# lbcb-sci/raven

Hardware: AMD Instinct MI355X
Metric: read Gbase/s through overlap+polish (higher is better)
Workload: dtype u32

## Files before the change

raven_amd/csrc/engine.h:

```cpp
#pragma once

#include <atomic>
#include <functional>
#include <memory>
#include <mutex>
#include <string>
#include <vector>

#include "common.h"

namespace rvn {

constexpr int kSketchTile = 1024;
constexpr int kMaxWindow = 256;

inline u64 next_reads_serial() {
  static std::atomic<u64> counter{0};
  return ++counter;
}

using BufFn = std::function<void(DevBuf&)>;
template <typename G>
void release_bufs(G& g) {
  g.for_each_buf([](DevBuf& b) { b.release(); });
// ... 34 lines not shown
  u64 m = 0;
  u64 u = 0;
  int table_bits = 0;
  int shift = 0;
  DevBuf s_val[2];
  DevBuf s_org[2];
  int cur = 0;
  DevBuf u_val;
  DevBuf u_start;
  DevBuf table;
  DevBuf direct;
  bool direct_built = false;
  u32 occurrence = 0xFFFFFFFFu;
  bool table_built = false;
  bool has_query_flags = false;
  bool all_query = false;
  u32 first = 0, last = 0;
  void for_each_buf(const BufFn& f) {
    f(s_val[0]), f(s_val[1]), f(s_org[0]), f(s_org[1]), f(u_val), f(u_start), f(table), f(direct);
  }
};

struct MapOut {
  u32 first = 0, last = 0;
  u64 n_query = 0;
  u64 n_matches = 0;
  u64 n_intervals = 0;
  u64 n_overlaps = 0;
  DevBuf ovl;
  DevBuf ovl_read_off;
  DevBuf filtered;
  bool has_anchors = false;
  DevBuf anchors;
  DevBuf anchor_off;
  DevBuf anchor_cnt;
  void for_each_buf(const BufFn& f) { f(ovl), f(ovl_read_off), f(filtered), f(anchors), f(anchor_off), f(anchor_cnt); }
};

struct StageTimes {
  enum { kSketch, kSort, kIndex, kFilter, kQuery, kMatch, kSegSort, kIntervals, kChain, kCompact, kMerge, kPile,
         kTruncate, kNum };
  double ms[kNum] = {};
  u64 launches[kNum] = {};
};

struct PileState;
struct PileRegion;
struct ResolveState;

struct EngineOptions {
  long long nw_budget_mb = 0;
  long long nw_group_walk = 0;
  long long nw_stripe_lanes = 0;
  long long ed_wide_lanes = 0;
  long long index_direct_min_keys = 0;
  long long poa_rows_min_windows = -1;
  long long io_threads = 0;
  long long io_slab_mb = 0;
  long long io_ring = 0;
  long long io_zlib = 0;
  long long arena_mb = 0;
  long long arena_margin_mb = 0;
  long long no_arena = 0;
  long long release_always = 0;
  long long polish_join = 0;
  long long polish_sketch_cache_mb = -1;
};
const char* engine_option_names();
long long* engine_option(EngineOptions& o, const char* name);

struct Engine;

struct SharedScratch {
  DevBuf tmp_a, tmp_b, tmp_c, tmp_d, tmp_e, tmp_f, scan_tmp, sort_tmp;
  void for_each_buf(const BufFn& f) {
    f(tmp_a), f(tmp_b), f(tmp_c), f(tmp_d), f(tmp_e), f(tmp_f), f(scan_tmp), f(sort_tmp);
  }
  void release() { release_bufs(*this); }
};

struct IoState {
  DevBuf text[2];
  std::vector<std::pair<std::unique_ptr<PinBuf>, bool>> pin;
  void for_each_buf(const BufFn& f) { f(text[0]), f(text[1]); }
  void release() { release_bufs(*this); }
};
struct LoadStats {
  u64 n_sequences = 0, n_bases = 0;
  int has_quality = 0;
  double parse_s = 0, device_s = 0, total_s = 0;
  u32 inflate_threads = 0, members = 0;
  int streaming = 0, restarted = 0;
};
void reads_load(Engine& e, const std::string& path, ReadsDev& R, std::vector<std::string>& names, LoadStats& st);

struct SketchState {
  Index index;
  Sketch index_sketch, query_sketch, raw_sketch;
  struct QueryReady {
    bool valid = false;
    u32 first = 0, last = 0;
    bool minhash = false;
  } query_ready;
  u64 join_query_count = 0;
  bool shard_sketch_minhash = false;
  DevBuf foreign_val, foreign_org;
// ... 61 lines not shown
void chain_allow_big_lds();

struct EditDistanceState {
  DevBuf cnt, sort, todo;
  void for_each_buf(const BufFn& f) { f(cnt), f(sort), f(todo); }
  void release() { release_bufs(*this); }
};
void edit_distance_batch(Engine& e, const ReadsDev& r, const u32* h_pairs, u32 n_pairs, u32* h_out, double* kernel_ms,
                         u64* cells);
void edit_distance_dev(Engine& e, const ReadsDev& r, const u32* d_pairs, u32 n_pairs, u32* d_out, const u32* d_kmax = nullptr,
                       bool wide_sweep = false);

struct PoaState {
  DevBuf scratch, scratch2;
  DevBuf sched, redo_w, redo_i;
  int mode = 0;
  u32 fallback_windows = 0;
  u32 fullmatrix_windows = 0;
  u32 wide_windows = 0;
  u32 narrow_windows = 0;
  unsigned long long phase_cycles[8] = {};
  u64 cells_full = 0, cells_band = 0, calls = 0;
  void for_each_buf(const BufFn& f) { f(scratch), f(scratch2), f(sched), f(redo_w), f(redo_i); }
  void release() { release_bufs(*this); }
};
void poa_consensus_batch(Engine& e, const u8* h_codes, const u8* h_quals, const u64* h_layer_off, const u32* h_begins,
                         const u32* h_ends, const u32* h_has_qual, const u32* h_win_off, u32 n_windows, int m, int n,
                         int g, int trim, u8* h_out, const u64* h_out_off, u32* h_out_len, u32* h_status,
                         double* device_ms);

void poa_banded_emulate(const u8* h_codes, const u8* h_quals, const u64* h_layer_off, const u32* h_begins,
                        const u32* h_ends, const u32* h_has_qual, const u32* h_win_off, u32 n_windows, int m, int n, int g,
                        int trim, u8* h_out, const u64* h_out_off, u32* h_out_len, u32* h_status, int variant);

struct PolishStats {
  u64 n_overlaps = 0, n_reads_used = 0, n_layers = 0, n_windows = 0, n_polished_windows = 0, n_failed_windows = 0;
  u64 n_dropped_layers = 0;
  double poa_ms = 0;
  double map_ms = 0, host_ms = 0, total_ms = 0;
  double align_ms = 0;
  u64 n_aligned = 0, n_align_retries = 0, align_band_cells = 0, align_store_bytes = 0;
};

struct NwStats {
  u64 n_aligned = 0, n_retries = 0, n_unaligned = 0, n_batches = 0;
  u64 band_cells = 0, sum_distance = 0, store_bytes = 0;
  double ms = 0;
};
struct NwState {
  struct Set {
    DevBuf hs, ck;
  } sets[4];
  DevBuf strip, jobs, res;
  double rate = -1.0;
  NwStats last;
  hipStream_t streams[5] = {};
  hipEvent_t ev[5] = {};
  hipStream_t side[3] = {};
  hipEvent_t side_ev[4] = {};
  void for_each_buf(const BufFn& f) {
    for (Set& s : sets) f(s.hs), f(s.ck);
    f(strip), f(jobs), f(res);
  }
  void release() { release_bufs(*this); }
  void open();
  void close();
  ~NwState() { close(); }
};
struct NwJob;
struct NwWindowRec;
struct NwPathSlots {
  std::vector<std::unique_ptr<DevBuf>> blocks;
  std::vector<u64> slot_end;
};
void nw_breakpoints(Engine& e, const ReadsDev& T, const ReadsDev& R, std::vector<NwJob>& jobs, u32 w, NwWindowRec* d_recs,
                    u64 n_recs, NwStats& st, std::vector<u32>* distances = nullptr, NwPathSlots* path = nullptr);
struct NwPaths {
  u32 n = 0, n_not_aligned = 0;
  u64 n_runs = 0, n_ops = 0;
  std::vector<u32> distances;
  DevBuf run_off, runs, op_off;
  double device_ms = 0;
};
void nw_align_paths(Engine& e, const ReadsDev& T, const ReadsDev& Q, std::vector<NwJob>& jobs, NwPaths& out);
void nw_paths_expand(Engine& e, const NwPaths& p, u8* d_ops);
int nw_breakpoints_host(const u64* t_words, u32 t_len, const u64* r_words, u32 r_len, u32 t_begin, u32 n, u32 q_begin, u32 m,
                        int rc, u32 w, u32 k, int force_R, NwWindowRec* recs, u32* distance, u32* band);
struct ShardState {
  DevBuf hist, off, ptrs;
  void for_each_buf(const BufFn& f) { f(hist), f(off), f(ptrs); }
  void release() { release_bufs(*this); }
};
void shard_split_minimizers(Engine& e, const u64* d_val, const u64* d_org, u64 n, u32 world, u64* d_val_out, u64* d_org_out,
                            u64* counts );
void shard_split_overlaps(Engine& e, const Overlap* d_ovl, u64 n, const u32* bounds , u32 world, u32 self,
                          Overlap* d_out, u64* counts );
u64 shard_count_flagged(Engine& e, const u64* d_org, u64 n);
void shard_adjacent_diff(Engine& e, const u64* d_seg, u64 n, u64* d_cnt);
void shard_regroup(Engine& e, u32 world, const u64* const* d_cnt, const u64* const* d_grp, const u64* const* d_pos,
                   const u64* n_src , u32 n_reads, u64* d_seg, u64* d_grp_out, u64* d_pos_out);
void shard_lhs_offsets(Engine& e, const Overlap* d_ovl, u64 n, u32 n_reads, u32* d_off);
struct PolishDirectOut {
  u8* out;
  const u64* off;
  u64* len;
};
struct PolishState {
  DevBuf best, best_t, idmap, recs, keep, win_cnt, win_off, win_fill, win_meta, first_window, keys, lays_tmp, lays, wins, out,
      len, status, ok, cons_off, stitched, quals, qual_off, misc;
  DevBuf tval, torg;
  struct KeptSketch {
    u32 first = 0, last = 0;
    Sketch sk;
  };
  u64 sketch_owner = 0;
// ... 357 lines not shown
```

raven_amd/csrc/engine.hip:

```cpp
#include <chrono>
#include <memory>

#include "abi.h"
#include "poa.h"

using namespace rvn;

static_assert(sizeof(rvn_overlap) == sizeof(rvn::Overlap), "overlap layout");

namespace {

thread_local std::string g_err;

const char* kStageNames[StageTimes::kNum] = {"sketch", "sort", "index", "filter", "query_sketch", "match",
                                             "seg_sort", "intervals", "chain", "compact", "merge", "pile",
                                             "truncate"};

}

namespace rvn {

void set_last_error(const std::string& msg) { g_err = msg; }
const std::string& last_error() { return g_err; }

// ... 16 lines not shown
    }
    Sketch& is = e.sketch.index_sketch;
    if (join && minhash) {
      sketch_minhash(e, r, e.sketch.raw_sketch, is);
      ix.all_query = true;
    } else if (!minhash) {
      is.val.swap(e.sketch.raw_sketch.val);
      is.org.swap(e.sketch.raw_sketch.org);
      is.read_off.swap(e.sketch.raw_sketch.read_off);
      is.first = first;
      is.last = last;
      is.count = e.sketch.raw_sketch.count;
      e.sketch.raw_sketch.count = 0;
      raw_handed_over = true;
    } else if (prefetch_query) {
      const Sketch& qs = e.sketch.query_sketch;
      const size_t vb = e.val64 ? 8 : 4;
      is.first = first;
      is.last = last;
      is.count = qs.count;
      is.val.reserve((qs.count + 1) * vb);
      is.org.reserve((qs.count + 1) * 8);
      if (qs.count) {
        RVN_HIP(hipMemcpyAsync(is.val.ptr, qs.val.ptr, qs.count * vb, hipMemcpyDeviceToDevice, e.stream));
        RVN_HIP(hipMemcpyAsync(is.org.ptr, qs.org.ptr, qs.count * 8, hipMemcpyDeviceToDevice, e.stream));
      }
    } else {
      sketch_minhash(e, r, e.sketch.raw_sketch, is);
    }
    t.stop();
  }
  for (u32 i = first; i < last; ++i) e.c_index_bases += r.h_len[i];
  e.c_index_min += e.sketch.index_sketch.count;
  index_build(e, e.sketch.index_sketch, !(e.sketch.index.has_query_flags || e.sketch.index.all_query));
  e.c_index_keys += e.sketch.index.u;
  if (raw_handed_over) {
    if (e.sketch.raw_sketch.val.cap < e.sketch.index_sketch.val.cap) e.sketch.raw_sketch.val.swap(e.sketch.index_sketch.val);
    if (e.sketch.raw_sketch.org.cap < e.sketch.index_sketch.org.cap) e.sketch.raw_sketch.org.swap(e.sketch.index_sketch.org);
  }
}

void fetch_values(Engine& e, const DevBuf& val, u64 n, u64* values) {
  if (!values || n == 0) return;
  if (e.val64) {
    RVN_HIP(hipMemcpy(values, val.ptr, n * 8, hipMemcpyDeviceToHost));
  } else {
    std::vector<u32> tmp(n);
    RVN_HIP(hipMemcpy(tmp.data(), val.ptr, n * 4, hipMemcpyDeviceToHost));
    for (u64 i = 0; i < n; ++i) values[i] = tmp[i];
  }
}

const char* engine_option_names() {
  return "nw_budget_mb, nw_group_walk, nw_stripe_lanes, ed_wide_lanes, index_direct_min_keys, poa_rows_min_windows, io_threads, io_slab_mb, io_ring, io_zlib, arena_mb, arena_margin_mb, "
         "no_arena, release_always, polish_join, polish_sketch_cache_mb";
}
long long* engine_option(EngineOptions& o, const char* name) {
  const std::string n(name ? name : "");
  if (n == "nw_budget_mb") return &o.nw_budget_mb;
  if (n == "nw_group_walk") return &o.nw_group_walk;
  if (n == "nw_stripe_lanes") return &o.nw_stripe_lanes;
  if (n == "ed_wide_lanes") return &o.ed_wide_lanes;
  if (n == "index_direct_min_keys") return &o.index_direct_min_keys;
  if (n == "poa_rows_min_windows") return &o.poa_rows_min_windows;
  if (n == "io_threads") return &o.io_threads;
  if (n == "io_slab_mb") return &o.io_slab_mb;
  if (n == "io_ring") return &o.io_ring;
  if (n == "io_zlib") return &o.io_zlib;
  if (n == "arena_mb") return &o.arena_mb;
  if (n == "arena_margin_mb") return &o.arena_margin_mb;
  if (n == "no_arena") return &o.no_arena;
  if (n == "release_always") return &o.release_always;
  if (n == "polish_join") return &o.polish_join;
  if (n == "polish_sketch_cache_mb") return &o.polish_sketch_cache_mb;
  return nullptr;
}

void engine_release_scratch(Engine& e) {
  if (e.stream) (void)rvn_stream_sync(e.stream);
  e.for_each_group([](auto& group) { group.release(); });
  delete e.pile_pool;
  e.pile_pool = nullptr;
}
void engine_release_scratch_if_tight(Engine& e, int stage_kind) {
  e.stage_kind = stage_kind;
  size_t free_b = 0, total_b = 0;
  if (hipMemGetInfo(&free_b, &total_b) != hipSuccess) return;
  const bool trace = knob("RVN_DEBUG_MEM") != nullptr;
  if (devpool::active()) {
    const size_t afree = devpool::free_total(), asize = devpool::size();
    const bool tight = afree * 4 < asize || ((e.oom_mask >> stage_kind) & 1u) || e.opt.release_always != 0;
    if (trace)
      std::fprintf(stderr, "[raven_hip] stage entry (kind %d): arena %.1f GB free of %.1f GB, driver %.1f GB free%s\n", stage_kind,
                   afree / 1e9, asize / 1e9, free_b / 1e9, tight ? " -> scratch released" : "");
    if (tight) engine_release_scratch(e);
    return;
  }
  const bool tight = free_b * 4 < total_b || e.opt.release_always != 0;
  if (trace)
    std::fprintf(stderr, "[raven_hip] stage entry (kind %d): %.1f GB free of %.1f GB%s\n", stage_kind, free_b / 1e9, total_b / 1e9,
                 tight ? " -> scratch released, arena started" : "");
  if (!tight) return;
  engine_release_scratch(e);
  if (e.opt.no_arena) return;
  if (hipMemGetInfo(&free_b, &total_b) != hipSuccess) return;
  size_t margin = std::max<size_t>(12ULL << 30, total_b / 16);
  if (e.opt.arena_margin_mb > 0) margin = static_cast<size_t>(e.opt.arena_margin_mb) << 20;
  if (e.opt.arena_mb > 0) margin = free_b > (static_cast<size_t>(e.opt.arena_mb) << 20) ? free_b - (static_cast<size_t>(e.opt.arena_mb) << 20) : free_b;
  if (free_b > margin + (1ULL << 30)) {
    const auto t0 = std::chrono::steady_clock::now();
    const bool ok = devpool::start(free_b - margin);
    if (trace)
      std::fprintf(stderr, "[raven_hip] arena of %.1f GB %s (%.0f ms)\n", (free_b - margin) / 1e9, ok ? "started" : "refused",
                   std::chrono::duration<double, std::milli>(std::chrono::steady_clock::now() - t0).count());
// ... 159 lines not shown
```

raven_amd/csrc/nwpath.hip:

```cpp
#include <algorithm>
#include <mutex>
#include <chrono>
#include <cmath>
#include <cstdio>
#include <cstdlib>
#include <exception>
#include <type_traits>
#include <vector>

#include "engine.h"
#include "nwpath.h"
#include "nwplan.h"
#include "nwsweep.h"
#include "nwtrace.h"
#include "wave.h"

namespace rvn {

namespace {

constexpr int kNwLaneStripCols = 16;
constexpr int kNwGroupLanes = 16;
constexpr u32 kNwGroupWalkMaxJobs = 8192;
constexpr u32 kSideSweepMaxWaves = 2048;
// ... 78 lines not shown
      const int o = __shfl_xor(n_steps_w, off, 64);
      n_steps_w = o > n_steps_w ? o : n_steps_w;
    }
    n_steps_w = __builtin_amdgcn_readfirstlane((n_steps_w + 15) & ~15);
    const int prev = lig == 0 ? gbase + (L > 0 ? L - 1 : 0) : lane - 1;
    const bool st_ok = has && lig < L;
    int n_g = (n_steps + kNwHsSteps - 1) / kNwHsSteps, n_q = n_steps / kNwCkSteps;
    if (STRIPED) {
      n_g = g0 + gps;
      n_q = qc0 + qps;
    }
    const u64 row = static_cast<u64>(L) * R;
    for (int t = t0; t <= n_steps_w; ++t) {
      int x = __shfl(ln.xf, prev, 64);
      if (STRIPED) {
        if (is_top) x = top.x(t);
        if (t == t_hand) sc_hand = ln.sc;
      }
      if (__ballot(ln.has_event(t)) != 0) {
        int sp = __shfl(ln.sc, prev, 64);
        if (STRIPED && is_top) sp = sc_in;
        if (ln.has_event(t)) ln.event(t, x, sp);
      }
      ln.step(t, x);
      if ((t & 15) == 0) {
        const int gi = (t >> 4) - 1;
        if (st_ok && gi < n_g) {
          u32* p = hs_j + static_cast<u64>(gi - g0) * row + static_cast<u64>(lig) * R;
#pragma unroll
          for (int r = 0; r < R; ++r) p[r] = ln.acc[r];
        }
        if ((t & 31) == 0) {
          const int qi = (t >> 5) - 1;
          if (st_ok && qi < n_q) {
            NwPm* p = ck_j + static_cast<u64>(qi - qc0) * row + static_cast<u64>(lig) * R;
#pragma unroll
            for (int r = 0; r < R; ++r) p[r] = NwPm{ln.Pv[r], ln.Mv[r]};
          }
        }
        ln.next_group(t);
        if (STRIPED && is_top) top.next_group(t);
      }
    }
    if (STRIPED && has && lig == lig_hand) hs_j[row * static_cast<u64>(gps)] = static_cast<u32>(sc_hand);
    const u32 res1 = group_max<G>(ln.result);
    if (has && lig == 0 && last) {
      const u32 res = res1 - 1u;
      result[ji] = res;
      status[ji] = (res1 != 0 && res <= k) ? 0u : 2u;
    }
  }
}

template <bool STRIP_LDS, int SC, class Out = NwWindowRec>
__global__ __launch_bounds__(64) void nw_trace_kernel(const NwJob* __restrict__ jobs, const u32* __restrict__ idx, u32 n_idx,
                                                      const u64* __restrict__ t_words, const u64* __restrict__ r_words,
                                                      const u32* __restrict__ hs, const NwPm* __restrict__ ck,
                                                      const u32* __restrict__ result, u32* __restrict__ status, u32 w,
                                                      Out* __restrict__ recs, u64* __restrict__ scratch) {
  __shared__ u64 s_pv[STRIP_LDS ? (SC + 1) * 64 : 1];
  __shared__ u64 s_mv[STRIP_LDS ? (SC + 1) * 64 : 1];
  __builtin_amdgcn_s_setprio(3);
  const u32 q = blockIdx.x * 64 + threadIdx.x;
  if (q >= n_idx) return;
  const u32 ji = idx[q];
  if (status[ji] != 0) return;
  const NwJob J = jobs[ji];
  const NwGeo geo = nw_geo_job(J);
  u64* g_pv = scratch + static_cast<u64>(blockIdx.x) * (2 * kNwStripCols * 64);
  const NwStripMem<64> mem{STRIP_LDS ? s_pv : g_pv, STRIP_LDS ? s_mv : g_pv + kNwStripCols * 64, static_cast<int>(threadIdx.x)};
  if constexpr (std::is_same<Out, u32>::value) {
    NwRunSink sink;
    sink.init(recs + J.bp_off, nw_slot_words(J.k));
    status[ji] = static_cast<u32>(nw_trace_job<64, SC, NwRunSink>(J, geo, t_words, r_words, hs + J.hs, ck + J.ckpt, mem, result[ji], w,
                                                                  nullptr, sink));
  } else {
    status[ji] = static_cast<u32>(nw_trace_job<64, SC>(J, geo, t_words, r_words, hs + J.hs, ck + J.ckpt, mem, result[ji], w, recs));
  }
}

template <int GL, class Out = NwWindowRec>
__global__ __launch_bounds__(64) void nw_trace_group_kernel(const NwJob* __restrict__ jobs, const u32* __restrict__ idx, u32 n_idx,
                                                            const u64* __restrict__ t_words, const u64* __restrict__ r_words,
                                                            const u32* __restrict__ hs, const NwPm* __restrict__ ck,
                                                            const u32* __restrict__ result, u32* __restrict__ status, u32 w,
                                                            Out* __restrict__ recs) {
  constexpr int NG = 64 / GL;
  __shared__ u64 s_pv[kNwStripCols * 64];
  __shared__ u64 s_mv[kNwStripCols * 64];
  __shared__ NwStripHead s_heads[64];
  __builtin_amdgcn_s_setprio(3);
  const int lane = static_cast<int>(threadIdx.x), grp = lane / GL, t = lane % GL;
  const u32 q = blockIdx.x * NG + static_cast<u32>(grp);
  if (q >= n_idx) return;
  const u32 ji = idx[q];
  if (status[ji] != 0) return;
  const NwJob J = jobs[ji];
  const NwGeo geo = nw_geo_job(J);
  constexpr bool kPath = std::is_same<Out, u32>::value;
  NwGroupWalk<64, GL, typename std::conditional<kPath, NwRunSink, NwNoSink>::type> G;
  if constexpr (kPath) {
    NwRunSink sink;
    sink.init(recs + J.bp_off, nw_slot_words(J.k));
    G.init(J, t_words, r_words, NwStripMem<64>{s_pv, s_mv, grp * GL}, s_heads + grp * GL, result[ji], w, nullptr, sink);
  } else {
    G.init(J, t_words, r_words, NwStripMem<64>{s_pv, s_mv, grp * GL}, s_heads + grp * GL, result[ji], w, recs);
  }
  int bad = 0;
  while (!G.done()) {
    G.fill(J, geo, hs + J.hs, ck + J.ckpt, t);
    __threadfence_block();
    __builtin_amdgcn_wave_barrier();
    bad = G.walk_batch(geo, t == 0);
    __threadfence_block();
    __builtin_amdgcn_wave_barrier();
    if (bad) break;
  }
  const int rcode = bad ? 1 : G.wk.finish(t == 0);
  if (t == 0) status[ji] = static_cast<u32>(rcode);
}

template <int R, int G, bool STRIPED = false>
void launch_sweep(Engine& e, hipStream_t s, const NwJob* d_jobs, const u32* d_idx, u32 n_idx, const ReadsDev& T, const ReadsDev& Rd,
                  u32* d_hs, NwPm* d_ck, u32* d_result, u32* d_status, u32* d_next, int stripe = 0) {
  if (n_idx == 0) return;
  constexpr u32 NG = 64 / G;
  const u32 bundles = (n_idx + NG - 1) / NG;
  const u32 per_simd = static_cast<u32>(sweep_waves_per_simd<R>());
  const u32 waves = std::min<u32>(bundles, 256u * 4u * (per_simd > 4 ? per_simd - 2 : per_simd));
  RVN_HIP(hipMemsetAsync(d_next, 0, 4, s));
  RVN_KLAUNCH_ON(kKNwForward, s, (nw_sweep_kernel<R, G, STRIPED><<<(waves + 3) / 4, 256, 0, s>>>(
                               d_jobs, d_idx, n_idx, T.packed.as<u64>(), Rd.packed.as<u64>(), d_hs, d_ck, d_result,
                               d_status, d_next, stripe)));
}


}

void NwState::open() {
  try {
    int prio_least = 0, prio_greatest = 0;
    RVN_HIP(hipDeviceGetStreamPriorityRange(&prio_least, &prio_greatest));
    for (int b = 0; b < 8; ++b) {
      hipStream_t& st2 = b < 5 ? streams[b] : side[b - 5];
      if (b >= 3 && prio_greatest != prio_least) RVN_HIP(hipStreamCreateWithPriority(&st2, hipStreamNonBlocking, prio_greatest));
      else RVN_HIP(hipStreamCreateWithFlags(&st2, hipStreamNonBlocking));
    }
    for (hipEvent_t& x : ev) RVN_HIP(hipEventCreateWithFlags(&x, hipEventDisableTiming));
    for (hipEvent_t& x : side_ev) RVN_HIP(hipEventCreateWithFlags(&x, hipEventDisableTiming));
  } catch (...) {
    close();
    throw;
  }
}
void NwState::close() {
  auto drop = [](auto& all, auto destroy) {
    for (auto& x : all) {
      if (x) (void)destroy(x);
      x = nullptr;
    }
  };
  drop(ev, hipEventDestroy);
  drop(streams, hipStreamDestroy);
  drop(side_ev, hipEventDestroy);
  drop(side, hipStreamDestroy);
}

namespace {

using clk = std::chrono::steady_clock;
double since(clk::time_point t) { return std::chrono::duration<double, std::milli>(clk::now() - t).count(); }

struct WalkGuard {
  Engine& e;
  ~WalkGuard() {
    if (!std::uncaught_exceptions()) return;
    for (hipStream_t st2 : e.nw.streams)
      if (st2) (void)hipStreamSynchronize(st2);
    for (hipStream_t st2 : e.nw.side)
      if (st2) (void)hipStreamSynchronize(st2);
    (void)hipStreamSynchronize(e.stream);
  }
};

u64 nw_budget(Engine& e) {
  size_t free_b = 0, total_b = 0;
  RVN_HIP(hipMemGetInfo(&free_b, &total_b));
  u64 held = 0;
  for (const NwState::Set& set : e.nw.sets) held += set.hs.cap + set.ck.cap;
  u64 budget = std::min<u64>((static_cast<u64>(free_b) + devpool::free_total()) / 4 + held, 64ULL << 30);
  if (e.opt.nw_budget_mb > 0) budget = static_cast<u64>(e.opt.nw_budget_mb) << 20;
  return std::max<u64>(budget, 64ULL << 20);
}

struct NwRun {
  Engine& e;
  const ReadsDev& T;
  const ReadsDev& Rd;
  std::vector<NwJob>& jobs;
  const u32 w;
  NwWindowRec* const d_recs;
  NwPathSlots* const path;
  NwStats& st;
  std::vector<u32>* const distances;
  const hipStream_t s;
  const u32 nj;
  const u64 budget;
  const u32 stripe_lanes;
  const bool trace_lds;
  const int group_walk;
  const bool one_stream, dbg_sync;
  const NwDevArrays dev;
  bool side_pending[3] = {false, false, false};
  bool set_used[4] = {false, false, false, false};
  struct Queued {
    std::vector<u32> order;
    NwPassDev dev;
    bool sweep_only;
    std::vector<u32> res, status;
  };
  std::vector<Queued> queued;
  std::vector<u8> early;
  std::vector<u32> h_result, h_status;
  std::vector<double> rates;
  std::vector<NwObs> obs;
  double h_plan = 0, h_order = 0, h_up = 0, h_res = 0;

  NwRun(Engine& e_, const ReadsDev& T_, const ReadsDev& Rd_, std::vector<NwJob>& jobs_, u32 w_, NwWindowRec* d_recs_, NwPathSlots* path_,
        NwStats& st_, std::vector<u32>* distances_)
      : e(e_), T(T_), Rd(Rd_), jobs(jobs_), w(w_), d_recs(d_recs_), path(path_), st(st_), distances(distances_), s(e_.stream),
        nj(static_cast<u32>(jobs_.size())), budget(nw_budget(e_)),
        stripe_lanes(e_.opt.nw_stripe_lanes > 0 && e_.opt.nw_stripe_lanes < 64 ? static_cast<u32>(e_.opt.nw_stripe_lanes) : 64u),
        trace_lds(!(knob("RVN_NW_TRACE_MEM") && std::atoi(knob("RVN_NW_TRACE_MEM")) == 1)),
        group_walk(static_cast<int>(e_.opt.nw_group_walk)), one_stream(knob("RVN_NW_ONE_STREAM") != nullptr),
        dbg_sync(knob("RVN_NW_DEBUG") && std::atoi(knob("RVN_NW_DEBUG")) >= 2), dev(arrays(e_, nj)), h_result(nj), h_status(nj) {
    rates.reserve(nj);
  }
  static NwDevArrays arrays(Engine& e, u32 nj) {
    const NwDevLayout at = nw_dev_layout(nj);
    NwJob* d_jobs = e.nw.jobs.get<NwJob>(at.n_jobs);
    return nw_dev_arrays(at, d_jobs, e.nw.res.get<u32>(at.n_words));
  }

  bool plan(NwJob& J, u64 k) const { return nw_plan(J, k, stripe_lanes, budget); }

  void join_side() {
    for (int x = 0; x < 3; ++x) {
      if (side_pending[x]) RVN_HIP(hipStreamWaitEvent(s, e.nw.side_ev[x], 0));
      side_pending[x] = false;
    }
  }

  struct ChunkDev {
    const NwPassDev& dev;
    int b;
    u32* hs;
    NwPm* ck;
    u64* d_strip;
    u32* d_slots;
  };

  template <class Out, class... Tail>
  void launch_walk_kernel(void (*kernel)(const NwJob*, const u32*, u32, const u64*, const u64*, const u32*, const NwPm*, const u32*, u32*, u32,
                                         Out*, Tail...),
                          u32 per_block, const ChunkDev& c, Out* d_out, hipStream_t wst, const u32* idx_w, u32 n_w, Tail... tail) {
    RVN_KLAUNCH_ON(kKNwTraceback, wst, (kernel<<<(n_w + per_block - 1) / per_block, 64, 0, wst>>>(
                                           c.dev.jobs, idx_w, n_w, T.packed.as<u64>(), Rd.packed.as<u64>(), c.hs, c.ck, c.dev.res,
                                           c.dev.status, w, d_out, tail...)));
  }
  template <class Out>
  void launch_walk_to(Out* d_out, const ChunkDev& c, hipStream_t wst, const u32* idx_w, u32 n_w) {
    if (group_walk == 2 || (group_walk != 1 && n_w <= kNwGroupWalkMaxJobs)) {
      launch_walk_kernel<Out>(nw_trace_group_kernel<kNwGroupLanes, Out>, 64 / kNwGroupLanes, c, d_out, wst, idx_w, n_w);
    } else if (trace_lds && (group_walk == 3 || (group_walk != 1 && n_w > 64u * 4u * 256u))) {
      launch_walk_kernel<Out, u64*>(nw_trace_kernel<true, kNwLaneStripCols, Out>, 64, c, d_out, wst, idx_w, n_w, nullptr);
    } else if (trace_lds) {
      launch_walk_kernel<Out, u64*>(nw_trace_kernel<true, kNwCkSteps, Out>, 64, c, d_out, wst, idx_w, n_w, nullptr);
    } else {
      launch_walk_kernel<Out, u64*>(nw_trace_kernel<false, kNwCkSteps, Out>, 64, c, d_out, wst, idx_w, n_w,
                                    c.d_strip + static_cast<size_t>(c.b) * ((e.nw.strip.cap / 32) & ~size_t(63)));
    }
  }
  void launch_walk(const ChunkDev& c, hipStream_t wst, const u32* idx_w, u32 n_w) {
    if (path) launch_walk_to(c.d_slots, c, wst, idx_w, n_w);
    else launch_walk_to(d_recs, c, wst, idx_w, n_w);
  }

  template <u32 X>
  void launch_variant(const ChunkDev& c, const NwChunk& C, const u32* idx_c, const bool* side) {
    constexpr int R = static_cast<int>(kNwVariants[X].R), G = static_cast<int>(kNwVariants[X].G);
    const u32 n = nw_count_of(C, X);
    launch_sweep<R, G>(e, side[X] ? e.nw.side[X % 3] : s, c.dev.jobs, idx_c + C.coff[X], n, T, Rd, c.hs, c.ck, c.dev.res, c.dev.status,
                       side[X] ? dev.side_next + X : dev.next);
    if (dbg_sync && n) {
      RVN_HIP(hipStreamSynchronize(s));
      std::fprintf(stderr, "[raven_hip] nw: sweep R=%d G=%d done, %u jobs\n", R, G, n);
    }
  }
  template <u32 X = kLevels - 1>
  void launch_variants(const ChunkDev& c, const NwChunk& C, const u32* idx_c, const bool* side) {
    launch_variant<X>(c, C, idx_c, side);
    if constexpr (X > 0) launch_variants<X - 1>(c, C, idx_c, side);
  }

  void enqueue(const std::vector<u32>& todo, bool sweep_only, NwLayout layout, const NwPassDev& pd, hipStream_t up, std::vector<u32>* left) {
    if (todo.empty()) return;
    auto t_h = clk::now();
    std::vector<u32> order = nw_order(jobs, todo);
    const NwChunks cut = nw_chunks(order, jobs, budget, layout, path && !sweep_only, left);
    const std::vector<NwChunk>& chunks = cut.chunks;
    st.band_cells += cut.band_cells;
    st.store_bytes = std::max<u64>(st.store_bytes, cut.store_bytes);
    for (int b = 0; b < 4; ++b) {
      const NwSetNeed need = nw_set_need(chunks, layout, b);
      if (!need.used) continue;
      (void)e.nw.sets[b].hs.get<u32>(need.hs_w + 4 * 64 * 8 + 16);
      (void)e.nw.sets[b].ck.get<NwPm>(need.ck_e + 16);
    }
    u64* d_strip = nullptr;
    if (!trace_lds) {
      size_t mc = 0;
      for (const NwChunk& C : chunks) mc = std::max(mc, C.c1 - C.c0);
      d_strip = e.nw.strip.get<u64>(static_cast<size_t>((mc + 63) / 64) * 2 * kNwStripCols * 64 * 4 + 64);
    }
    u32* d_slots = nullptr;
    if (path && !sweep_only) {
      path->blocks.emplace_back(new DevBuf());
      d_slots = path->blocks.back()->get<u32>(cut.slot_w + 16);
      for (u32 i : order) path->slot_end[i] = reinterpret_cast<u64>(d_slots + jobs[i].bp_off + nw_slot_words(jobs[i].k) - 1);
    }
    h_order += since(t_h);
    t_h = clk::now();
    if (pd.compact) {
      std::vector<NwJob> hj(order.size());
      std::vector<u32> iota(order.size());
      for (size_t x = 0; x < order.size(); ++x) {
        hj[x] = jobs[order[x]];
        iota[x] = static_cast<u32>(x);
      }
      RVN_HIP(hipMemcpyAsync(pd.jobs, hj.data(), hj.size() * sizeof(NwJob), hipMemcpyHostToDevice, up));
      RVN_HIP(hipMemcpyAsync(pd.idx, iota.data(), iota.size() * 4, hipMemcpyHostToDevice, up));
      RVN_HIP(rvn_stream_sync(up));
    } else {
      RVN_HIP(hipMemcpyAsync(pd.jobs, jobs.data(), static_cast<size_t>(nj) * sizeof(NwJob), hipMemcpyHostToDevice, up));
      RVN_HIP(hipMemcpyAsync(pd.idx, order.data(), order.size() * 4, hipMemcpyHostToDevice, up));
      RVN_HIP(rvn_stream_sync(up));
    }
    h_up += since(t_h);
    for (size_t ci = 0; ci < chunks.size(); ++ci) {
      const NwChunk& C = chunks[ci];
      const int b = nw_set_of(ci, layout);
      const ChunkDev c{pd, b, e.nw.sets[b].hs.as<u32>(), e.nw.sets[b].ck.as<NwPm>(), d_strip, d_slots};
      const u32* idx_c = pd.idx + C.c0;
      const u32 cn = static_cast<u32>(C.c1 - C.c0);
      if (set_used[b]) RVN_HIP(hipStreamWaitEvent(s, e.nw.ev[b], 0));
      hipStream_t ts = one_stream ? s : e.nw.streams[b];
      bool side[kLevels] = {};
      bool side_used[3] = {false, false, false};
      {
        u32 n_levels = 0;
        for (u32 x = 0; x < kLevels; ++x) n_levels += nw_count_of(C, x) ? 1u : 0u;
        if (n_levels >= 2 && !one_stream && !dbg_sync)
          for (u32 x = 0; x < kLevels; ++x) {
            const u32 per_wave = 64 / kNwVariants[x].G;
            const u32 bundles = (nw_count_of(C, x) + per_wave - 1) / per_wave;
            side[x] = nw_count_of(C, x) && bundles <= kSideSweepMaxWaves;
            if (side[x]) side_used[x % 3] = true;
          }
        if (side_used[0] || side_used[1] || side_used[2]) {
          RVN_HIP(hipEventRecord(e.nw.side_ev[3], s));
          for (int y = 0; y < 3; ++y)
            if (side_used[y]) RVN_HIP(hipStreamWaitEvent(e.nw.side[y], e.nw.side_ev[3], 0));
        }
      }
      if (const u32 n_str = nw_count_of(C, kStriped)) {
        const u32* idx_s = idx_c + C.coff[kStriped];
        std::vector<u32> n_stripes(n_str);
        for (u32 x = 0; x < n_str; ++x) n_stripes[x] = static_cast<u32>(nw_geo_job(jobs[order[C.c0 + C.coff[kStriped] + x]]).n_stripes);
        for (u32 stp = 0;; ++stp) {
          u32 n_st = 0;
          while (n_st < n_str && n_stripes[n_st] > stp) ++n_st;
          if (n_st == 0) break;
          launch_sweep<static_cast<int>(kNwStripedVariant.R), static_cast<int>(kNwStripedVariant.G), true>(
              e, s, pd.jobs, idx_s, n_st, T, Rd, c.hs, c.ck, pd.res, pd.status, dev.next, static_cast<int>(stp));
          if (dbg_sync) {
            RVN_HIP(hipStreamSynchronize(s));
            std::fprintf(stderr, "[raven_hip] nw: stripe %u done, %u jobs\n", stp, n_st);
          }
        }
      }
      launch_variants(c, C, idx_c, side);
      for (int y = 0; y < 3; ++y)
        if (side_used[y]) {
          RVN_HIP(hipEventRecord(e.nw.side_ev[y], e.nw.side[y]));
          side_pending[y] = true;
        }
      ++st.n_batches;
      if (sweep_only) continue;
      if (!one_stream) {
        RVN_HIP(hipEventRecord(e.nw.ev[4], s));
        RVN_HIP(hipStreamWaitEvent(ts, e.nw.ev[4], 0));
        for (int y = 0; y < 3; ++y)
          if (side_used[y]) RVN_HIP(hipStreamWaitEvent(ts, e.nw.side_ev[y], 0));
      }
      launch_walk(c, ts, idx_c, cn);
      if (!one_stream) {
        RVN_HIP(hipEventRecord(e.nw.ev[b], ts));
        set_used[b] = true;
      }
      if (dbg_sync) {
        RVN_HIP(hipStreamSynchronize(ts));
        std::fprintf(stderr, "[raven_hip] nw: trace done, %u jobs\n", cn);
      }
    }
    queued.push_back(Queued{std::move(order), pd, sweep_only, {}, {}});
  }

  void collect(std::vector<u32>& again) {
    again.clear();
    join_side();
    for (int b = 0; b < 4; ++b) {
      if (set_used[b]) RVN_HIP(hipStreamWaitEvent(s, e.nw.ev[b], 0));
      set_used[b] = false;
    }
    for (Queued& q : queued) {
      if (q.dev.compact) {
        q.res.resize(q.order.size());
        q.status.resize(q.order.size());
        RVN_HIP(hipMemcpyAsync(q.res.data(), q.dev.res, q.order.size() * 4, hipMemcpyDeviceToHost, s));
        RVN_HIP(hipMemcpyAsync(q.status.data(), q.dev.status, q.order.size() * 4, hipMemcpyDeviceToHost, s));
      }
    }
    RVN_HIP(hipMemcpyAsync(h_result.data(), dev.all.res, static_cast<size_t>(nj) * 4, hipMemcpyDeviceToHost, s));
    RVN_HIP(hipMemcpyAsync(h_status.data(), dev.all.status, static_cast<size_t>(nj) * 4, hipMemcpyDeviceToHost, s));
    RVN_HIP(rvn_stream_sync(s));
    auto t_h = clk::now();
    for (const Queued& q : queued)
      if (q.dev.compact)
        for (size_t x = 0; x < q.order.size(); ++x) {
          h_result[q.order[x]] = q.res[x];
          h_status[q.order[x]] = q.status[x];
        }
    for (size_t qi = 0; qi < queued.size(); ++qi) {
      const Queued& q = queued[qi];
// ... 562 lines not shown
```

raven_amd/csrc/nwplan.h:

```cpp
#pragma once

#include <algorithm>
#include <cmath>
#include <vector>

#include "nwpath.h"

namespace rvn {

struct NwVariant {
  u32 R, G;
};
constexpr NwVariant kNwVariants[] = {{1, 4}, {1, 8}, {1, 16}, {1, 32}, {1, 64}, {2, 64}, {4, 64}, {8, 64}};
constexpr u32 kLevels = sizeof(kNwVariants) / sizeof(kNwVariants[0]);
constexpr NwVariant kNwStripedVariant = kNwVariants[kLevels - 1];
constexpr u32 kNwMaxStripes = 8;
constexpr u32 kStriped = kLevels;
constexpr u32 kClasses = kLevels + 1;
constexpr u32 kHeadMax = 4096;

inline u32 kcap_of(u32 n, u32 m, u32 R, u32 G) {
  const u32 d = n > m ? n - m : m - n;
  const u64 room = static_cast<u64>(G) * (64ULL * R + 1) - 64ULL * R;
  if (room < d) return 0;
// ... 105 lines not shown
    C.c0 = c0;
    size_t c1 = c0;
    while (c1 < order.size()) {
      NwJob& J = jobs[order[c1]];
      const u64 hw = need[c1].hw, ce = need[c1].ce;
      const u64 share = (chunks.empty() && layout != kRotating) ? budget / 12 : budget / 3;
      if (c1 > c0 && (C.hs_w + hw) * 4 + (C.ck_e + ce) * 16 > share) break;
      J.hs = C.hs_w;
      J.ckpt = C.ck_e;
      if (slots) {
        J.bp_off = out.slot_w;
        out.slot_w += nw_slot_words(J.k);
      }
      C.hs_w += hw;
      C.ck_e += ce;
      out.band_cells += need[c1].cells;
      C.coff[need[c1].level + 1]++;
      ++c1;
    }
    u32 run_off = 0, cnt[kClasses];
    for (u32 x = 0; x < kClasses; ++x) cnt[x] = C.coff[x + 1];
    for (int x = static_cast<int>(kClasses) - 1; x >= 0; --x) {
      C.coff[x] = run_off;
      run_off += cnt[x];
    }
    C.coff[kClasses] = run_off;
    C.c1 = c1;
    out.store_bytes = std::max<u64>(out.store_bytes, C.hs_w * 4 + C.ck_e * 16);
    chunks.push_back(C);
    c0 = c1;
    if (layout == kHeadOnly) break;
  }
  if (layout == kHeadOnly && !chunks.empty() && chunks[0].c1 < order.size()) {
    for (size_t x = chunks[0].c1; x < order.size(); ++x) left->push_back(order[x]);
    order.resize(chunks[0].c1);
  }
  return out;
}

struct NwSetNeed {
  bool used;
  u64 hs_w, ck_e;
};
inline NwSetNeed nw_set_need(const std::vector<NwChunk>& chunks, NwLayout layout, int b) {
  NwSetNeed need{false, 0, 0};
  for (size_t ci = 0; ci < chunks.size(); ++ci) {
    if (nw_set_of(ci, layout) != b) continue;
    need.used = true;
    need.hs_w = std::max(need.hs_w, chunks[ci].hs_w);
    need.ck_e = std::max(need.ck_e, chunks[ci].ck_e);
  }
  return need;
}

struct NwObs {
  double len, d;
};
struct NwThresholdModel {
  double mu = -1, va = 0, vb = 0;
  void fit(const std::vector<NwObs>& obs) {
    if (obs.size() < 256) return;
    double sl = 0, sd = 0;
    for (const NwObs& o : obs) {
      sl += o.len;
      sd += o.d;
    }
    mu = sd / sl;
    std::vector<double> zs;
    for (const NwObs& o : obs) zs.push_back(std::fabs(o.d - mu * o.len) / std::sqrt(o.len));
    std::vector<double> zsorted = zs;
    std::sort(zsorted.begin(), zsorted.end());
    const double zcut = zsorted[static_cast<size_t>(zsorted.size() * 0.98)];
    double s11 = 0, s12 = 0, s22 = 0, t1 = 0, t2 = 0, sr = 0, sn = 0;
    for (size_t x = 0; x < obs.size(); ++x) {
      if (zs[x] > zcut) continue;
      const double L = obs[x].len * 1e-3, r2 = (obs[x].d - mu * obs[x].len) * (obs[x].d - mu * obs[x].len);
      s11 += L * L;
      s12 += L * L * L;
      s22 += L * L * L * L;
      t1 += r2 * L;
      t2 += r2 * L * L;
      sr += r2 / L;
      sn += 1;
    }
    const double det = s11 * s22 - s12 * s12;
    double a = -1, b = -1;
    if (det > 1e-9 * s11 * s22) {
      a = (t1 * s22 - t2 * s12) / det;
      b = (t2 * s11 - t1 * s12) / det;
    }
    if (!(a >= 0) || !(b >= 0)) {
      a = sn > 0 ? sr / sn : mu * 1e3;
      b = 0;
    }
    va = std::max(a * 1e-3, 0.25 * mu);
    vb = b * 1e-6;
  }
  u64 threshold(double len, double rate) const {
    const double z = 4.5;
    return mu > 0 ? static_cast<u64>(mu * len + z * std::sqrt(va * len + vb * len * len)) + 6 : static_cast<u64>(rate * len) + 16;
  }
  static u64 pilot_threshold(double len, double rate) { return static_cast<u64>((rate * 1.25 + 0.02) * len) + 16; }
};

inline u32 nw_job_len(const NwJob& J) { return std::max(J.n, J.m); }

// ... 88 lines not shown
```

Baseline: 1.444.

## Pack variable-width R=1 NW sweep jobs into shared wavefronts via host bin-packing

Adds a packed sweep kernel in which one 64-lane wavefront processes several R=1 alignment jobs of different lane widths side by side. A host-side planner sorts the jobs by step count, bin-packs them into bundles by width and uploads a bundle table. By default this applies only to chunks where the per-variant R=1 launches would need more than the side-sweep wave limit. The aim is to cut wasted lanes and per-variant kernel launches from small-width jobs that previously got fixed G-lane groups. In exchange it adds host packing cost, an extra upload, and shuffle and ballot overhead inside the kernel.

```diff
diff --git a/raven_amd/csrc/engine.h b/raven_amd/csrc/engine.h
--- a/raven_amd/csrc/engine.h
+++ b/raven_amd/csrc/engine.h
@@ -110,6 +110,7 @@
   long long nw_budget_mb = 0;
   long long nw_group_walk = 0;
   long long nw_stripe_lanes = 0;
+  long long nw_pack = 1;
   long long ed_wide_lanes = 0;
   long long index_direct_min_keys = 0;
   long long poa_rows_min_windows = -1;
@@ -277,6 +278,7 @@
     DevBuf hs, ck;
   } sets[4];
   DevBuf strip, jobs, res;
+  DevBuf pack;
   double rate = -1.0;
   NwStats last;
   hipStream_t streams[5] = {};
@@ -285,7 +287,7 @@
   hipEvent_t side_ev[4] = {};
   void for_each_buf(const BufFn& f) {
     for (Set& s : sets) f(s.hs), f(s.ck);
-    f(strip), f(jobs), f(res);
+    f(strip), f(jobs), f(res), f(pack);
   }
   void release() { release_bufs(*this); }
   void open();
diff --git a/raven_amd/csrc/engine.hip b/raven_amd/csrc/engine.hip
--- a/raven_amd/csrc/engine.hip
+++ b/raven_amd/csrc/engine.hip
@@ -92,7 +92,7 @@
 }
 
 const char* engine_option_names() {
-  return "nw_budget_mb, nw_group_walk, nw_stripe_lanes, ed_wide_lanes, index_direct_min_keys, poa_rows_min_windows, io_threads, io_slab_mb, io_ring, io_zlib, arena_mb, arena_margin_mb, "
+  return "nw_budget_mb, nw_group_walk, nw_stripe_lanes, nw_pack, ed_wide_lanes, index_direct_min_keys, poa_rows_min_windows, io_threads, io_slab_mb, io_ring, io_zlib, arena_mb, arena_margin_mb, "
          "no_arena, release_always, polish_join, polish_sketch_cache_mb";
 }
 long long* engine_option(EngineOptions& o, const char* name) {
@@ -100,6 +100,7 @@
   if (n == "nw_budget_mb") return &o.nw_budget_mb;
   if (n == "nw_group_walk") return &o.nw_group_walk;
   if (n == "nw_stripe_lanes") return &o.nw_stripe_lanes;
+  if (n == "nw_pack") return &o.nw_pack;
   if (n == "ed_wide_lanes") return &o.ed_wide_lanes;
   if (n == "index_direct_min_keys") return &o.index_direct_min_keys;
   if (n == "poa_rows_min_windows") return &o.poa_rows_min_windows;
diff --git a/raven_amd/csrc/nwpath.hip b/raven_amd/csrc/nwpath.hip
--- a/raven_amd/csrc/nwpath.hip
+++ b/raven_amd/csrc/nwpath.hip
@@ -154,6 +154,90 @@
   }
 }
 
+__global__ __launch_bounds__(256) __attribute__((amdgpu_waves_per_eu(sweep_waves_per_simd<1>())))
+void nw_sweep_packed_kernel(const NwJob* __restrict__ jobs, const u32* __restrict__ idx, u32 n_idx, const u32* __restrict__ b_off,
+                            const u32* __restrict__ mem, u32 n_bundles, const u64* __restrict__ t_words,
+                            const u64* __restrict__ r_words, u32* __restrict__ hs, NwPm* __restrict__ ck, u32* __restrict__ result,
+                            u32* __restrict__ status, u32* __restrict__ next) {
+  __shared__ u64 s_peq[4][4 * 64];
+  const int lane = lane_id();
+  u64* peq = s_peq[threadIdx.x >> 6];
+  for (;;) {
+    u32 b = atomicAdd(next, lane == 0 ? 1u : 0u);
+    b = static_cast<u32>(__builtin_amdgcn_readfirstlane(static_cast<int>(b)));
+    if (b >= n_bundles) break;
+    const u32 m0 = b_off[b], m1 = b_off[b + 1];
+    const int n_mem = static_cast<int>(m1 - m0 < 64u ? m1 - m0 : 64u);
+    u32 mem_pos = 0, mem_at = 0;
+    if (lane < n_mem) {
+      mem_pos = mem[2 * (static_cast<u64>(m0) + static_cast<u32>(lane))];
+      mem_at = mem[2 * (static_cast<u64>(m0) + static_cast<u32>(lane)) + 1];
+    }
+    u32 q = ~0u;
+    int lane0 = lane, Lm = 0;
+    for (int x = 0; x < n_mem; ++x) {
+      const u32 at = static_cast<u32>(__shfl(static_cast<int>(mem_at), x, 64)), pos = static_cast<u32>(__shfl(static_cast<int>(mem_pos), x, 64));
+      const int l0 = static_cast<int>(at & 0xFFu), lm = static_cast<int>(at >> 8);
+      if (lane >= l0 && lane < l0 + lm) {
+        q = pos;
+        lane0 = l0;
+        Lm = lm;
+      }
+    }
+    const bool has = q < n_idx && lane0 + Lm <= 64;
+    const int lig = lane - lane0;
+    NwSweepLane<1, 64> ln;
+    u32 ji = 0;
+    int L = 0, n_steps = 0;
+    u32* hs_l = hs;
+    NwPm* ck_l = ck;
+    if (has) {
+      ji = idx[q];
+      const NwJob J = jobs[ji];
+      const NwGeo geo = nw_geo(J.n, J.m, J.k, 1);
+      n_steps = lig < geo.L ? geo.n_steps : 0;
+      ln.init(J, t_words, r_words, geo, lig, peq, lane);
+      L = geo.L;
+      hs_l = hs + J.hs + lig;
+      ck_l = ck + J.ckpt + lig;
+    } else {
+      ln.init_idle(peq, lane);
+    }
+    int n_steps_w = n_steps;
+#pragma unroll
+    for (int off = 32; off > 0; off >>= 1) {
+      const int o = __shfl_xor(n_steps_w, off, 64);
+      n_steps_w = o > n_steps_w ? o : n_steps_w;
+    }
+    n_steps_w = __builtin_amdgcn_readfirstlane((n_steps_w + 15) & ~15);
+    const int prev = (has && lig == 0) ? lane + L - 1 : (has ? lane - 1 : lane);
+    for (int t = 1; t <= n_steps_w; ++t) {
+      const int x = __shfl(ln.xf, prev, 64);
+      if (__ballot(ln.has_event(t)) != 0) {
+        const int sp = __shfl(ln.sc, prev, 64);
+        if (ln.has_event(t)) ln.event(t, x, sp);
+      }
+      ln.step(t, x);
+      if ((t & 15) == 0) {
+        const u32 at = static_cast<u32>((t >> 4) - 1) * static_cast<u32>(L);
+        if (t < n_steps + 16) hs_l[at] = ln.acc[0];
+        if ((t & 31) == 0 && t <= n_steps) ck_l[(at - static_cast<u32>(L)) >> 1] = NwPm{ln.Pv[0], ln.Mv[0]};
+        ln.next_group(t);
+      }
+    }
+    const bool first = n_steps > 0 && prev >= lane;
+    const u64 ring = (L >= 64 ? ~0ULL : ((1ULL << L) - 1ULL)) << lane;
+    const u64 got = __ballot(ln.result != 0) & ring;
+    const int src = got ? static_cast<int>(__builtin_ctzll(got)) : lane;
+    const u32 held = static_cast<u32>(__shfl(static_cast<int>(ln.result), src, 64));
+    if (first) {
+      const u32 res1 = got ? held : 0u, res = res1 - 1u;
+      result[ji] = res;
+      status[ji] = (res1 != 0 && res <= jobs[ji].k) ? 0u : 2u;
+    }
+  }
+}
+
 template <bool STRIP_LDS, int SC, class Out = NwWindowRec>
 __global__ __launch_bounds__(64) void nw_trace_kernel(const NwJob* __restrict__ jobs, const u32* __restrict__ idx, u32 n_idx,
                                                       const u64* __restrict__ t_words, const u64* __restrict__ r_words,
@@ -236,6 +320,17 @@
                                d_status, d_next, stripe)));
 }
 
+void launch_sweep_packed(Engine& e, hipStream_t s, const NwJob* d_jobs, const u32* d_idx, u32 n_idx, const u32* d_off, const u32* d_mem,
+                         u32 n_bundles, const ReadsDev& T, const ReadsDev& Rd, u32* d_hs, NwPm* d_ck, u32* d_result, u32* d_status,
+                         u32* d_next) {
+  if (n_bundles == 0) return;
+  const u32 per_simd = static_cast<u32>(sweep_waves_per_simd<1>());
+  const u32 waves = std::min<u32>(n_bundles, 256u * 4u * (per_simd - 2));
+  RVN_HIP(hipMemsetAsync(d_next, 0, 4, s));
+  RVN_KLAUNCH_ON(kKNwForward, s, (nw_sweep_packed_kernel<<<(waves + 3) / 4, 256, 0, s>>>(
+                               d_jobs, d_idx, n_idx, d_off, d_mem, n_bundles, T.packed.as<u64>(), Rd.packed.as<u64>(), d_hs, d_ck,
+                               d_result, d_status, d_next)));
+}
 
 }
 
@@ -312,7 +407,10 @@
   const bool trace_lds;
   const int group_walk;
   const bool one_stream, dbg_sync;
+  const int pack_mode;
+  bool packs(const NwChunk& C) const { return pack_mode == 2 || (pack_mode == 1 && nw_variant_waves(C) > kSideSweepMaxWaves); }
   const NwDevArrays dev;
+  u32* const d_pack;
   bool side_pending[3] = {false, false, false};
   bool set_used[4] = {false, false, false, false};
   struct Queued {
@@ -335,13 +433,23 @@
         stripe_lanes(e_.opt.nw_stripe_lanes > 0 && e_.opt.nw_stripe_lanes < 64 ? static_cast<u32>(e_.opt.nw_stripe_lanes) : 64u),
         trace_lds(!(knob("RVN_NW_TRACE_MEM") && std::atoi(knob("RVN_NW_TRACE_MEM")) == 1)),
         group_walk(static_cast<int>(e_.opt.nw_group_walk)), one_stream(knob("RVN_NW_ONE_STREAM") != nullptr),
-        dbg_sync(knob("RVN_NW_DEBUG") && std::atoi(knob("RVN_NW_DEBUG")) >= 2), dev(arrays(e_, nj)), h_result(nj), h_status(nj) {
+        dbg_sync(knob("RVN_NW_DEBUG") && std::atoi(knob("RVN_NW_DEBUG")) >= 2), pack_mode(static_cast<int>(e_.opt.nw_pack)), dev(arrays(e_, nj)),
+        d_pack(e_.nw.pack.get<u32>(nw_pack_words(static_cast<size_t>(nj_of(jobs_)) + 1) + 2 * nw_pack_words(kHeadMax))), h_result(nj),
+        h_status(nj) {
     rates.reserve(nj);
   }
   static NwDevArrays arrays(Engine& e, u32 nj) {
     const NwDevLayout at = nw_dev_layout(nj);
     NwJob* d_jobs = e.nw.jobs.get<NwJob>(at.n_jobs);
     return nw_dev_arrays(at, d_jobs, e.nw.res.get<u32>(at.n_words));
+  }
+
+  static u32 nj_of(const std::vector<NwJob>& jobs) { return static_cast<u32>(jobs.size()); }
+  u32* pack_of(const NwPassDev& pd) const {
+    const size_t all_w = nw_pack_words(static_cast<size_t>(nj) + 1);
+    if (pd.jobs == dev.head.jobs) return d_pack + all_w;
+    if (pd.jobs == dev.retry.jobs) return d_pack + all_w + nw_pack_words(kHeadMax);
+    return d_pack;
   }
 
   bool plan(NwJob& J, u64 k) const { return nw_plan(J, k, stripe_lanes, budget); }
@@ -400,9 +508,9 @@
     }
   }
   template <u32 X = kLevels - 1>
-  void launch_variants(const ChunkDev& c, const NwChunk& C, const u32* idx_c, const bool* side) {
-    launch_variant<X>(c, C, idx_c, side);
-    if constexpr (X > 0) launch_variants<X - 1>(c, C, idx_c, side);
+  void launch_variants(const ChunkDev& c, const NwChunk& C, const u32* idx_c, const bool* side, u32 lowest) {
+    if (X >= lowest) launch_variant<X>(c, C, idx_c, side);
+    if constexpr (X > 0) launch_variants<X - 1>(c, C, idx_c, side, lowest);
   }
 
   void enqueue(const std::vector<u32>& todo, bool sweep_only, NwLayout layout, const NwPassDev& pd, hipStream_t up, std::vector<u32>* left) {
@@ -431,6 +539,34 @@
       d_slots = path->blocks.back()->get<u32>(cut.slot_w + 16);
       for (u32 i : order) path->slot_end[i] = reinterpret_cast<u64>(d_slots + jobs[i].bp_off + nw_slot_words(jobs[i].k) - 1);
     }
+    std::vector<u32> pack_tab, chunk_b0(chunks.size() + 1, 0);
+    u32* const d_tab = pack_of(pd);
+    bool any_packed = false;
+    for (const NwChunk& C : chunks) any_packed = any_packed || packs(C);
+    if (any_packed) {
+      std::vector<u32> offs{0}, mem;
+      mem.reserve(2 * order.size());
+      std::vector<NwPack> made(chunks.size());
+      parallel_for(chunks.size(), 1, [this, &made, &order, &chunks](size_t c0, size_t c1) {
+        for (size_t ci = c0; ci < c1; ++ci)
+          if (packs(chunks[ci])) made[ci] = nw_pack(jobs, order, chunks[ci]);
+      });
+      for (size_t ci = 0; ci < chunks.size(); ++ci) {
+        const NwPack& P = made[ci];
+        const u32 m_base = static_cast<u32>(mem.size() / 2);
+        for (size_t b = 1; b < P.off.size(); ++b) offs.push_back(m_base + P.off[b]);
+        for (const NwPackMember& M : P.mem) {
+          mem.push_back(M.pos);
+          mem.push_back(M.lane0 | (M.L << 8));
+        }
+        chunk_b0[ci + 1] = static_cast<u32>(offs.size() - 1);
+      }
+      pack_tab.swap(offs);
+      pack_tab.insert(pack_tab.end(), mem.begin(), mem.end());
+      if (pack_tab.size() > nw_pack_words(order.size())) throw HipError("[raven_hip] alignment path: bundle table beyond its bound (internal error)");
+      RVN_HIP(hipMemcpyAsync(d_tab, pack_tab.data(), pack_tab.size() * 4, hipMemcpyHostToDevice, up));
+    }
+    const u32* const d_pack_mem = d_tab + chunk_b0[chunks.size()] + 1;
     h_order += since(t_h);
     t_h = clk::now();
     if (pd.compact) {
@@ -459,16 +595,20 @@
       hipStream_t ts = one_stream ? s : e.nw.streams[b];
       bool side[kLevels] = {};
       bool side_used[3] = {false, false, false};
+      const u32 lowest = packs(C) ? kNwPackTop + 1 : 0;
+      const u32 n_packed = chunk_b0[ci + 1] - chunk_b0[ci];
       {
-        u32 n_levels = 0;
-        for (u32 x = 0; x < kLevels; ++x) n_levels += nw_count_of(C, x) ? 1u : 0u;
-        if (n_levels >= 2 && !one_stream && !dbg_sync)
-          for (u32 x = 0; x < kLevels; ++x) {
+        u32 n_levels = n_packed ? 1u : 0u;
+        for (u32 x = lowest; x < kLevels; ++x) n_levels += nw_count_of(C, x) ? 1u : 0u;
+        if (n_levels >= 2 && !one_stream && !dbg_sync) {
+          for (u32 x = lowest; x < kLevels; ++x) {
             const u32 per_wave = 64 / kNwVariants[x].G;
             const u32 bundles = (nw_count_of(C, x) + per_wave - 1) / per_wave;
             side[x] = nw_count_of(C, x) && bundles <= kSideSweepMaxWaves;
             if (side[x]) side_used[x % 3] = true;
           }
+          if (n_packed && n_packed <= kSideSweepMaxWaves) side[kNwPackTop] = side_used[kNwPackTop % 3] = true;
+        }
         if (side_used[0] || side_used[1] || side_used[2]) {
           RVN_HIP(hipEventRecord(e.nw.side_ev[3], s));
           for (int y = 0; y < 3; ++y)
@@ -491,7 +631,16 @@
           }
         }
       }
-      launch_variants(c, C, idx_c, side);
+      launch_variants(c, C, idx_c, side, lowest);
+      if (n_packed) {
+        const bool beside = side[kNwPackTop];
+        launch_sweep_packed(e, beside ? e.nw.side[kNwPackTop % 3] : s, pd.jobs, pd.idx, static_cast<u32>(order.size()), d_tab + chunk_b0[ci],
+                            d_pack_mem, n_packed, T, Rd, c.hs, c.ck, pd.res, pd.status, beside ? dev.side_next + kNwPackTop : dev.next);
+        if (dbg_sync) {
+          RVN_HIP(hipStreamSynchronize(s));
+          std::fprintf(stderr, "[raven_hip] nw: packed sweep done, %u bundles\n", n_packed);
+        }
+      }
       for (int y = 0; y < 3; ++y)
         if (side_used[y]) {
           RVN_HIP(hipEventRecord(e.nw.side_ev[y], e.nw.side[y]));
diff --git a/raven_amd/csrc/nwplan.h b/raven_amd/csrc/nwplan.h
--- a/raven_amd/csrc/nwplan.h
+++ b/raven_amd/csrc/nwplan.h
@@ -181,6 +181,101 @@
   }
   return need;
 }
+
+constexpr u32 kNwPackTop = 4;
+static_assert(kNwVariants[kNwPackTop].R == 1 && kNwVariants[kNwPackTop].G == 64 && kNwVariants[kNwPackTop + 1].R > 1,
+              "the packed classes are the R = 1 variants");
+struct NwPackMember {
+  u32 pos;
+  u32 lane0;
+  u32 L;
+};
+struct NwPack {
+  std::vector<u32> off;
+  std::vector<NwPackMember> mem;
+  std::vector<u32> steps;
+};
+
+inline std::vector<u32> nw_by_descending(const std::vector<u32>& key) {
+  const size_t n = key.size();
+  std::vector<u32> idx(n), tmp(n);
+  u32 top = 0;
+  for (size_t x = 0; x < n; ++x) {
+    idx[x] = static_cast<u32>(x);
+    top = std::max(top, key[x]);
+  }
+  for (int sh = 0; sh < 32 && (top >> sh) != 0; sh += 11) {
+    u32 cnt[2049] = {};
+    for (size_t x = 0; x < n; ++x) cnt[(((top - key[idx[x]]) >> sh) & 2047u) + 1]++;
+    for (int c = 0; c < 2048; ++c) cnt[c + 1] += cnt[c];
+    for (size_t x = 0; x < n; ++x) tmp[cnt[((top - key[idx[x]]) >> sh) & 2047u]++] = idx[x];
+    idx.swap(tmp);
+  }
+  return idx;
+}
+
+inline NwPack nw_pack(const std::vector<NwJob>& jobs, const std::vector<u32>& order, const NwChunk& C) {
+  NwPack out;
+  out.off.push_back(0);
+  const size_t p0 = C.c0 + C.coff[kNwPackTop], n = C.c1 - p0;
+  if (n == 0) return out;
+  std::vector<u32> lanes(n), steps(n);
+  parallel_for(n, 16384, [&jobs, &order, &lanes, &steps, p0](size_t x0, size_t x1) {
+    for (size_t x = x0; x < x1; ++x) {
+      const NwJob& J = jobs[order[p0 + x]];
+      const NwGeo g = nw_geo(J.n, J.m, J.k, 1);
+      lanes[x] = std::min<u32>(static_cast<u32>(g.L), 64);
+      steps[x] = static_cast<u32>(g.n_steps);
+    }
+  });
+  const std::vector<u32> by = nw_by_descending(steps);
+  u32 woff[66] = {}, cur[65];
+  for (size_t x = 0; x < n; ++x) woff[lanes[x] + 1]++;
+  for (u32 v = 0; v < 65; ++v) woff[v + 1] += woff[v];
+  for (u32 v = 0; v < 65; ++v) cur[v] = woff[v];
+  std::vector<u32> of_width(n);
+  for (size_t x = 0; x < n; ++x) of_width[cur[lanes[by[x]]]++] = by[x];
+  for (u32 v = 0; v < 65; ++v) cur[v] = woff[v];
+  std::vector<u32> b_off{0}, b_steps;
+  std::vector<NwPackMember> b_mem;
+  b_mem.reserve(n);
+  for (u32 widest = 64;;) {
+    while (widest >= 1 && cur[widest] == woff[widest + 1]) --widest;
+    if (widest < 1) break;
+    u32 lane0 = 0, longest = 0;
+    for (u32 v = widest; v >= 1;) {
+      if (cur[v] == woff[v + 1]) {
+        --v;
+        continue;
+      }
+      const u32 x = of_width[cur[v]++];
+      b_mem.push_back(NwPackMember{static_cast<u32>(p0 + x), lane0, v});
+      lane0 += v;
+      longest = std::max(longest, steps[x]);
+      v = std::min(v, 64 - lane0);
+    }
+    b_off.push_back(static_cast<u32>(b_mem.size()));
+    b_steps.push_back(longest);
+  }
+  out.mem.reserve(n);
+  for (u32 b : nw_by_descending(b_steps)) {
+    out.mem.insert(out.mem.end(), b_mem.begin() + b_off[b], b_mem.begin() + b_off[b + 1]);
+    out.off.push_back(static_cast<u32>(out.mem.size()));
+    out.steps.push_back(b_steps[b]);
+  }
+  return out;
+}
+
+inline u32 nw_variant_waves(const NwChunk& C) {
+  u32 waves = 0;
+  for (u32 x = 0; x <= kNwPackTop; ++x) {
+    const u32 per_wave = 64 / kNwVariants[x].G;
+    waves += (nw_count_of(C, x) + per_wave - 1) / per_wave;
+  }
+  return waves;
+}
+
+inline size_t nw_pack_words(size_t n_jobs) { return 3 * n_jobs + 1; }
 
 struct NwObs {
   double len, d;
```

New measurement: 1.427. 0.988x the previous value.
